# SerezD/gen_adversarial

Hardware: AMD Instinct MI355X
Metric: purified images/sec (attack+encode+decode) (higher is better)
Workload: dtype f32 storage; contractions as 3x bf16 MFMA (hi/lo split), fp32 accumulate; 1 GPU; configs[1]: NVAE purify + VGG-11, 64x64, PGD-Linf step (fwd + input-grad), bs 256 images/GPU x EoT 32 = 8192 defender rows per step, alphas ours_cosine_no_preprocessing_ids.yaml x0.7, assumed NVAE config (C=32, 3x8 groups, 20 latents); images_per_gpu=256, eot=32, rows_per_gpu=8192, chunk_rows=1024, streams=2, parallelism=image-sharded x1

## Files before the change

### gen_adversarial_amd/csrc/dec_cell.hip

```cpp
#include "ga_common.h"
#include "dec_cell_common.h"

namespace ga {

template <int C, int TMW, int NW>
__global__ void __launch_bounds__(64 * NW, NW / 4) dec_cell_fwd_kernel(const ga_dec_cell_desc d, const dc_geom gm) {
    constexpr int NTHR = 64 * NW;
    constexpr int M = 32 * TMW * NW, KS = C / 16, NT = C / 32, SW = M / (NTHR / 8);
    constexpr int BH = TMW == 2 ? 2 : 1, BW = SW / BH;
    using WA = w_chunk<C, true, NTHR>;
    using WB = w_chunk<C, false, NTHR>;
    extern __shared__ __attribute__((aligned(16))) float smem[];
    float* wS = smem;
    float* P1 = smem + 25 * DC_CH;
    const int plane_px = (M >> gm.lhw) * gm.PH * gm.PW;
    __bf16* P2h = reinterpret_cast<__bf16*>(P1 + plane_px * DC_PS);
    __bf16* P2l = P2h + M * DC_LDB;
    __bf16* W1h = P2l + M * DC_LDB;
    __bf16* W1l = W1h + WA::ELEMS;
    __bf16* W2h = W1l + WA::ELEMS;
    __bf16* W2l = W2h + WB::ELEMS;

    const int tid = threadIdx.x, lane = tid & 63, wave = tid >> 6, lrow = lane & 31, lh = lane >> 5;
    const int c4 = tid & 7, strip = tid >> 3;
// ... 211 lines not shown

    WA wa, wq;
    wa.issue(g1h, g1l, C, 0, tid);
    wq.issue(g2h, g2l, C, 0, tid);
    const size_t tap_o = (size_t)(tid < 200 ? (tid >> 3) : 0) * d.Hd + 4 * c4;

    for (int i = tid; i < plane_px * (DC_PS / 4); i += NTHR) reinterpret_cast<floatx4*>(P1)[i] = zero;

    bf16x8 xh[TMW][KS], xl[TMW][KS], gh[TMW][KS], gl[TMW][KS];
#pragma unroll
    for (int i = 0; i < TMW; ++i) {
        const size_t gp = pix0 + wb + i * 32 + lrow;
        const size_t n = gp >> gm.lhw;
        const size_t xp = d.act_rep > 1 ? (((n / (size_t)d.act_rep) << gm.lhw) + (gp & (size_t)(gm.HW - 1))) : gp;
#pragma unroll
        for (int ks = 0; ks < KS; ++ks) {
            const int k = ks * 16 + 8 * lh;
            const float* p = d.x + xp * C + k;
            split8(*reinterpret_cast<const floatx4*>(p), *reinterpret_cast<const floatx4*>(p + 4), xh[i][ks], xl[i][ks]);
            const float* q = d.dout + gp * C + k;
            const float* s = d.pro_scale + n * C + k;
            const float* t = d.pro_shift + n * C + k;
            const floatx4 a = *reinterpret_cast<const floatx4*>(q) * *reinterpret_cast<const floatx4*>(s) + *reinterpret_cast<const floatx4*>(t);
            const floatx4 b = *reinterpret_cast<const floatx4*>(q + 4) * *reinterpret_cast<const floatx4*>(s + 4) + *reinterpret_cast<const floatx4*>(t + 4);
            split8(a, b, gh[i][ks], gl[i][ks]);
        }
    }
    const int p0 = tile_pixel<BH, BW>(strip, gm);
    const int ctr = plane_idx(p0, gm);
    const int win = ctr - 2 * gm.PW - 2;
    int prow[TMW][4];
#pragma unroll
    for (int i = 0; i < TMW; ++i)
#pragma unroll
        for (int q = 0; q < 4; ++q) prow[i][q] = plane_idx(wb + i * 32 + 8 * q + 4 * lh, gm) * DC_PS + lrow;

    const int nch = d.Hd / DC_CH;
    DC_T0
#pragma unroll 1
    for (int ch = 0; ch < nch; ++ch) {
        const int h0 = ch * DC_CH;
        wa.store(W1h, W1l, tid);
        wq.store(W2h, W2l, tid);
        __syncthreads();
        DC_T(0)
        const float b1v = d.b1[h0 + lrow];
        const floatx4 bd4 = *reinterpret_cast<const floatx4*>(d.bd + h0 + 4 * c4);
        const floatx4 taps = *reinterpret_cast<const floatx4*>(d.wd + tap_o + h0);
        const floatx4 tapsT = *reinterpret_cast<const floatx4*>(d.wd_bwd + tap_o + h0);
        __builtin_amdgcn_sched_barrier(0);
        floatx16 t1[TMW];
#pragma unroll
        for (int i = 0; i < TMW; ++i)
#pragma unroll
            for (int r = 0; r < 16; ++r) t1[i][r] = 0.f;
        gemm_resident<TMW, KS>(t1, xh, xl, W1h + lrow * WA::PITCH + 8 * lh, W1l + lrow * WA::PITCH + 8 * lh);
#pragma unroll
        for (int i = 0; i < TMW; ++i)
#pragma unroll
            for (int r = 0; r < 16; ++r) {
                const int row = wb + i * 32 + (r & 3) + 8 * (r >> 2) + 4 * lh;
                const float v = t1[i][r] + b1v;
                const float sg = fast_sigmoid(v);
                P4[row * DC_PS + lrow] = sg * (1.0f + v * (1.0f - sg));
                P1[prow[i][r >> 2] + (r & 3) * DC_PS] = v * sg;
            }
        if (tid < 200) {
            *reinterpret_cast<floatx4*>(wS + (tid >> 3) * DC_CH + 4 * c4) = taps;
            *reinterpret_cast<floatx4*>(wT + (tid >> 3) * DC_CH + 4 * c4) = tapsT;
        }
        DC_T(1)
        __syncthreads();
        DC_T(2)
        floatx4 g2[SW];
        dw_tile<BH, BW>(g2, P1 + win * DC_PS + 4 * c4, wS + 4 * c4, gm.PW);
        DC_T(3)
        floatx16 g[TMW];
#pragma unroll
        for (int i = 0; i < TMW; ++i)
#pragma unroll
            for (int r = 0; r < 16; ++r) g[i][r] = 0.f;
        {
            const __bf16* w2h = W2h + lrow * WA::PITCH + 8 * lh;
            const __bf16* w2l = W2l + lrow * WA::PITCH + 8 * lh;
            constexpr int KPJ = KS / SW;
            bf16x8 bh[KPJ], bl[KPJ];
#pragma unroll
            for (int k = 0; k < KPJ; ++k) {
                bh[k] = *reinterpret_cast<const bf16x8*>(w2h + k * 16);
                bl[k] = *reinterpret_cast<const bf16x8*>(w2l + k * 16);
            }
#pragma unroll
            for (int j = 0; j < SW; ++j) {
                bf16x8 nh[KPJ], nl[KPJ];
                if (j + 1 < SW) {
#pragma unroll
                    for (int k = 0; k < KPJ; ++k) {
                        nh[k] = *reinterpret_cast<const bf16x8*>(w2h + ((j + 1) * KPJ + k) * 16);
                        nl[k] = *reinterpret_cast<const bf16x8*>(w2l + ((j + 1) * KPJ + k) * 16);
                    }
                }
#pragma unroll
                for (int k = 0; k < KPJ; ++k)
#pragma unroll
                    for (int i = 0; i < TMW; ++i) mfma3(g[i], gh[i][j * KPJ + k], gl[i][j * KPJ + k], bh[k], bl[k]);
#pragma unroll
                for (int e = 0; e < 4; ++e) g2[j][e] = dsilu_f(g2[j][e] + bd4[e]);
                interleave_mfma_valu<KPJ * TMW * 3, 44>();
                __builtin_amdgcn_sched_barrier(0);
                if (j + 1 < SW) {
#pragma unroll
                    for (int k = 0; k < KPJ; ++k) { bh[k] = nh[k]; bl[k] = nl[k]; }
                }
            }
        }
        DC_T(4)
        __syncthreads();
        DC_T(5)
        {
            const int h1 = min(h0 + DC_CH, (nch - 1) * DC_CH);
            wa.issue(g1h, g1l, C, h1, tid);
            wq.issue(g2h, g2l, C, h1, tid);
        }
#pragma unroll
        for (int i = 0; i < TMW; ++i)
#pragma unroll
            for (int r = 0; r < 16; ++r) P1[prow[i][r >> 2] + (r & 3) * DC_PS] = g[i][r];
        __syncthreads();
        DC_T(6)
#pragma unroll
        for (int j = 0; j < SW; ++j) {
            floatx4* q = reinterpret_cast<floatx4*>(P1 + (ctr + (j / BW) * gm.PW + (j % BW)) * DC_PS + 4 * c4);
            *q = *q * g2[j];
        }
        __syncthreads();
        DC_T(7)
        {
            floatx4 a[SW];
            dw_tile<BH, BW>(a, P1 + win * DC_PS + 4 * c4, wT + 4 * c4, gm.PW);
#pragma unroll
            for (int j = 0; j < SW; ++j) {
                const int pj = p0 + (j / BW) * gm.W + (j % BW);
                const floatx4 u = *reinterpret_cast<const floatx4*>(P4 + pj * DC_PS + 4 * c4);
                *reinterpret_cast<floatx4*>(d.y + (pix0 + pj) * d.Hd + h0 + 4 * c4) = a[j] * u;
            }
        }
        DC_T(8)
        __syncthreads();
        DC_T(9)
    }
    DC_TEND
}

static int log2_exact(int v) {
    int l = 0;
    while ((1 << l) < v) ++l;
    return (1 << l) == v ? l : -1;
}

constexpr size_t DC_LDS_MAX = 160 * 1024;

static int dc_tile_pixels(int C) { return C == 128 ? 256 : C == 256 ? 128 : 0; }

static size_t dc_lds_bytes(int C, int M, int H, int W, bool bwd) {
    const size_t plane_px = (size_t)(M / (H * W)) * (H + 4) * (W + 4);
    const size_t rows32 = (size_t)2 * 32 * (C + 8) * 2, cols32 = (size_t)2 * C * 40 * 2;
    return bwd ? (size_t)(50 * DC_CH + plane_px * DC_PS + (size_t)M * DC_PS) * 4 + 2 * rows32
               : (size_t)(25 * DC_CH + plane_px * DC_PS) * 4 + (size_t)2 * M * DC_LDB * 2 + rows32 + cols32;
}

template <int C, int TMW, int NW>
static int launch_dec_cell(const ga_dec_cell_desc& d, const dc_geom& gm, hipStream_t stream) {
    constexpr int M = 32 * TMW * NW;
    const size_t lds = dc_lds_bytes(C, M, d.H, d.W, d.backward != 0);
    const dim3 grid((unsigned)((size_t)d.N * d.H * d.W / M));
    if (d.backward) {
        static dyn_lds_cache attr;
        if (!ensure_dyn_lds(attr, reinterpret_cast<const void*>(&dec_cell_bwd_kernel<C, TMW, NW>), lds)) return GA_E_LAUNCH;
        hipLaunchKernelGGL((dec_cell_bwd_kernel<C, TMW, NW>), grid, dim3(64 * NW), lds, stream, d, gm);
    } else {
        static dyn_lds_cache attr;
        if (!ensure_dyn_lds(attr, reinterpret_cast<const void*>(&dec_cell_fwd_kernel<C, TMW, NW>), lds)) return GA_E_LAUNCH;
        hipLaunchKernelGGL((dec_cell_fwd_kernel<C, TMW, NW>), grid, dim3(64 * NW), lds, stream, d, gm);
    }
    return check_launch();
}

}

#ifdef GA_DC_TRACE
extern "C" int ga_debug_dc_trace_read(unsigned long long* out, int n) {
    return hipMemcpyFromSymbol(out, HIP_SYMBOL(ga::ga_dc_trace_buf), (size_t)n * 8) == hipSuccess ? GA_OK : GA_E_LAUNCH;
}
#endif

extern "C" int ga_dec_cell_supported(int N, int H, int W, int C, int Hd) {
    using namespace ga;
    const int M = dc_tile_pixels(C);
    if (!M || N <= 0 || H <= 0 || W <= 0 || Hd <= 0 || Hd % DC_CH) return 0;
    if (log2_exact(W) < 0 || log2_exact(H) < 0) return 0;
    const long HW = (long)H * W;
    if (HW > M || M % HW || W % (M / 32)) return 0;
    if (C == 128 && H % 2) return 0;
    if (((long)N * HW) % M) return 0;
    return dc_lds_bytes(C, M, H, W, true) <= DC_LDS_MAX && dc_lds_bytes(C, M, H, W, false) <= DC_LDS_MAX;
}

extern "C" int ga_dec_cell(const ga_dec_cell_desc* dp, void* stream_) {
    ga::clear_stale_error();
    using namespace ga;
    if (!dp) return GA_E_BADARG;
    const ga_dec_cell_desc& d = *dp;
    if (!d.x || !d.w1_hi || !d.w1_lo || !d.b1 || !d.wd || !d.bd || !d.w2_hi || !d.w2_lo || !d.y) return GA_E_BADARG;
    if (d.backward ? (!d.dout || !d.pro_scale || !d.pro_shift || !d.wd_bwd) : !d.b2) return GA_E_BADARG;
    if (!ga_dec_cell_supported(d.N, d.H, d.W, d.C, d.Hd)) return GA_E_UNSUPPORTED;
    if (d.act_rep > 1 && (!d.backward || d.N % d.act_rep)) return GA_E_BADARG;
    const void* ptrs[] = {d.x, d.w1_hi, d.w1_lo, d.wd, d.wd_bwd, d.bd, d.w2_hi, d.w2_lo, d.dout, d.pro_scale, d.pro_shift, d.y};
    for (const void* p : ptrs) if (p && !aligned16(p)) return GA_E_ALIGN;
    dc_geom gm;
    gm.W = d.W; gm.HW = d.H * d.W; gm.lw = log2_exact(d.W); gm.lhw = log2_exact(gm.HW); gm.PW = d.W + 4; gm.PH = d.H + 4;
    hipStream_t stream = reinterpret_cast<hipStream_t>(stream_);
    if (d.C == 128) return d.variant == 1 ? launch_dec_cell<128, 1, 8>(d, gm, stream) : launch_dec_cell<128, 2, 4>(d, gm, stream);
    if (d.C == 256) return launch_dec_cell<256, 1, 4>(d, gm, stream);
    return GA_E_UNSUPPORTED;
}
```

### gen_adversarial_amd/engine.py

```python
from __future__ import annotations

import ctypes as C
import json
import os
from typing import Dict, List, Optional, Sequence

import torch

from . import _lib as L
from . import folding as F
from .nvae_spec import DecCellSpec, EncCellSpec, NVAESpec, build_spec
from .e4e_spec import E4ESpec
from .resnet_spec import ResNetSpec
from .vgg_spec import VggSpec
from .engine_core import (IMG_LD, RES_SCALE, TILES, TUNE_FILE, WS_FLOATS, Act, WeightStore, _ptr, conv_key,
                          candidate_tiles, resolve_tile, tile_candidates, tune_cache)
from .engine_classifiers import ClassifierBuilder
from .engine_e4e import E4EBuilder
from .engine_avae import AvaeBuilder
from .engine_ndvae import NdvaeBuilder
from .engine_nvae import NvaeBuilder
from .engine_stylegan import StyleGanBuilder
from .engine_trans import TransBuilder


def expand_alpha_rows(alphas, rows: int, rep: int, pairs: bool) -> torch.Tensor:
    t = alphas.detach().to('cpu', torch.float64) if isinstance(alphas, torch.Tensor) else torch.tensor(alphas, dtype=torch.float64)
    if t.dim() != 2:
        raise ValueError(f'a [K, n] table of alpha vectors expected, got shape {tuple(t.shape)}')
    K = t.shape[0]
    if K != rows:
        if K < 1 or rep % K or rows % rep:
            raise ValueError(f'{K} candidates do not divide the {rep} rows per image')
        t = t.repeat_interleave(rep // K, dim=0).repeat(rows // rep, 1)
    if not pairs:
        return t.to(torch.float32)
    return torch.stack([t.to(torch.float32), (1.0 - t).to(torch.float32)], dim=2).reshape(rows, -1)


class Engine(NvaeBuilder, NdvaeBuilder, AvaeBuilder, ClassifierBuilder, E4EBuilder, StyleGanBuilder, TransBuilder):
    fuse_dec_cells = os.environ.get('GA_FUSE_DEC_CELL', '1') != '0'
    fuse_min_workgroups = 0 if os.environ.get('GA_FUSE_DEC_CELL') == 'force' else 160
    fuse_halo_cells = os.environ.get('GA_FUSE_HALO_CELL', '0') == '1'
    dec_cell_variant = int(os.environ.get('GA_DEC_CELL_VARIANT', '1'))

    def __init__(self, nvae_sd, nvae_cfg: dict, resolution, vgg_sd, vgg_spec: VggSpec, rows: int, rep: int,
                 alphas: Sequence[float], temperature: float = 0.6, noise_eps: float = 0.0,
                 device: str = 'cuda:0', need_backward: bool = True, dry_run: bool = False,
                 store: Optional[WeightStore] = None, precision: str = 'bf16x3', blur: bool = False,
                 share_encoder: bool = False, cot_rep: int = 1, alpha_rows: bool = False, alpha_grad: bool = False):
        if rows % rep:
            raise ValueError('rows must be a multiple of the EoT repeat')
        self.device = torch.device(device)
        self.dry_run = dry_run
        if self.device.type != 'cuda' and not dry_run:
            raise RuntimeError('the HIP engine needs a GPU device; there is no CPU fallback '
                               '(dry_run=True only builds and validates the plans)')
        if precision not in ('fp32', 'bf16x3'):
            raise ValueError("precision must be 'fp32' (exact f32 MFMA) or 'bf16x3' (3 bf16 MFMAs per product)")
        self.precision = precision
        self.store = store if store is not None else WeightStore(self.device)
        self.has_nvae = nvae_sd is not None
        self.spec: Optional[NVAESpec] = build_spec(nvae_cfg, resolution) if self.has_nvae else None
        self.resolution = tuple(resolution)
        self.vspec = vgg_spec
        self.rows, self.rep = rows, rep
        self.alphas = [float(a) for a in alphas]
        if self.has_nvae and len(self.alphas) != len(self.spec.groups):
            raise ValueError(f'{len(self.spec.groups)} interpolation alphas expected, got {len(self.alphas)}')
        self.temperature = float(temperature)
        self.noise_eps = float(noise_eps)
        self.blur = bool(blur)
        self._init_alpha_rows(alpha_rows)
        self.share_encoder = bool(share_encoder) and rep > 1 and self.noise_eps == 0.0 and nvae_sd is not None
        self.enc_rows = rows // rep if self.share_encoder else rows
        self.need_backward = need_backward
        if cot_rep < 1:
            raise ValueError('cot_rep (cotangents per forward row of the backward plan) must be at least 1')
        if cot_rep > 1 and not (isinstance(vgg_spec, VggSpec) or (isinstance(vgg_spec, ResNetSpec) and not self.has_nvae)):
            raise ValueError('cot_rep > 1 (K-cotangent backward) is built for the defenders in front of a VGG classifier, for the VGG '
                             'classifier itself and for a bare ResNet / ResNeXt classifier (input noise and blur included); still '
                             'refused: a purifier in front of a ResNet / ResNeXt classifier, and the e4e classifier spec')
        self.cot_rep = int(cot_rep)
        self._init_alpha_grad(alpha_grad)
        self._init_plans()
        self._build(nvae_sd, vgg_sd)

    @classmethod
    def bare(cls, rows: int, device='cuda:0', precision: str = 'bf16x3', store: Optional[WeightStore] = None,
             dry_run: bool = False, rep: int = 1, resolution=None, alphas: Sequence[float] = (), noise_eps: float = 0.0,
             need_backward: bool = True, blur: bool = False, share_encoder: bool = False, alpha_rows: bool = False,
             cot_rep: int = 1, alpha_grad: bool = False) -> "Engine":
        if cot_rep < 1:
            raise ValueError('cot_rep (cotangents per forward row of the backward plan) must be at least 1')
        self = cls.__new__(cls)
        self.device, self.dry_run, self.precision = torch.device(device), dry_run, precision
        if self.device.type != 'cuda' and not dry_run:
            raise RuntimeError('the HIP engine needs a GPU device; there is no CPU fallback')
        self.store = store if store is not None else WeightStore(self.device)
        if rows % rep:
            raise ValueError('rows must be a multiple of the EoT repeat')
        self.has_nvae, self.spec, self.vspec, self.resolution = False, None, None, (tuple(resolution) if resolution else None)
        self.rows, self.rep, self.alphas, self.temperature = rows, rep, [float(a) for a in alphas], 1.0
        self.noise_eps, self.blur = float(noise_eps), bool(blur)
        self._init_alpha_rows(alpha_rows)
        self.share_encoder = bool(share_encoder) and rep > 1 and self.noise_eps == 0.0
        self.enc_rows = rows // rep if self.share_encoder else rows
        self.need_backward, self.image_s2d, self.cot_rep = need_backward, False, int(cot_rep)
        self._init_alpha_grad(alpha_grad)
        self._init_plans()
        self._scratch = {}
        self.eps, self.purified, self.dpurified, self._purified_grad_nhwc = [], None, None, None
        return self

    def finish(self):
        self._finish(0)
        return self

    def _init_plans(self):
        self.bytes = 0
        self.acts = {}
        self.version = 0
        self._sampler_descs = []
        self._keep = []
        self._conv_w = {}
        self.fwd = L.Plan()
        self.bwd = L.Plan()
        self._bwd_steps = []

    def _init_alpha_rows(self, alpha_rows: bool):
        self.alpha_rows, self.alpha_table = bool(alpha_rows), None
        if self.alpha_rows and self.rep > 1 and self.noise_eps != 0.0:
            raise ValueError('a per-row alpha engine with rep > 1 shares the encoder pass of an image between its rows: '
                             'not available with input noise (initial_noise_eps > 0)')

    def _init_alpha_grad(self, alpha_grad: bool):
        self.alpha_grad, self.alpha_grad_rows = bool(alpha_grad), None
        if self.alpha_grad and self.cot_rep > 1:
            raise ValueError('alpha_grad reduces one cotangent per row: not available together with cot_rep > 1')
        if self.alpha_grad and not self.need_backward:
            raise ValueError('alpha_grad lives in the backward plan: not available with need_backward=False')

    def alpha_grads(self) -> torch.Tensor:
        if self.alpha_grad_rows is None:
            raise RuntimeError('engine was built without the alpha-gradient ops (alpha_grad=True)')
        return self.alpha_grad_rows

    def _alloc_alpha_table(self, n: int, pairs: bool) -> torch.Tensor:
        self._alpha_pairs = pairs
        self.alpha_table = self.alloc((self.rows, (2 if pairs else 1) * n))
        self.alpha_table.copy_(expand_alpha_rows([self.alphas], self.rows, self.rows, pairs))
        return self.alpha_table

    def alloc(self, shape) -> torch.Tensor:
        t = torch.zeros(shape, dtype=torch.float32, device=self.device)
        self.bytes += t.numel() * 4
        self._keep.append(t)
        return t

    def dev(self, t: torch.Tensor) -> torch.Tensor:
        t = t.to(self.device, dtype=torch.float32).contiguous()
        self._keep.append(t)
        self.bytes += t.numel() * 4
        return t

    def devd(self, key: str, fn) -> dict:
        return self.store.get(key, fn)

    def conv(self, plan, name, x, w, y, *, cin=None, cout=None, bias=None, K=1, sn=1, sd=1, pad=0,
             x2=None, pro_scale=None, pro_shift=None, pro_act=0, pro_per_row=0,
             addend=None, addend_bcast=False, addend2=None, dact_x=None, dact_scale=None, dact_shift=None, dact_act=0,
             in_hw=None, out_hw=None, n=None, KH=None, KW=None, anchored=False, explicit_out=False,
             ldx=None, ldy=None, ldadd=None, flags=0, precise=False):
        d = L.ConvDesc()
        N, Hi, Wi, Cx = x.shape
        d.x, d.ldx = _ptr(x), (ldx or Cx)
        d.C1 = cin if cin is not None else Cx
        if x2 is not None:
            d.x2, d.ldx2, d.C2 = _ptr(x2), x2.shape[3], x2.shape[3]
        d.w, d.bias = _ptr(w), _ptr(bias)
        if self.precision == 'bf16x3' and not self.dry_run and not precise:
            hi, lo = self.store.split(w)
            d.w_hi, d.w_lo = _ptr(hi), _ptr(lo)
            self._conv_w[id(d)] = w
        d.pro_scale, d.pro_shift, d.pro_act, d.pro_per_row = _ptr(pro_scale), _ptr(pro_shift), pro_act, pro_per_row
        No, Ho, Wo, Cy = y.shape
        d.y, d.ldy = _ptr(y), (ldy or Cy)
        d.flags = flags
        d.Cout = cout if cout is not None else Cy
        if addend is not None:
            d.addend, d.ldadd, d.addend_bcast_n = _ptr(addend), (ldadd or addend.shape[-1]), int(addend_bcast)
        if addend2 is not None:
            d.addend2, d.ldadd2 = _ptr(addend2), addend2.shape[-1]
        if dact_x is not None:
            d.dact_x, d.lddact = _ptr(dact_x), dact_x.shape[-1]
            d.dact_scale, d.dact_shift, d.dact_act = _ptr(dact_scale), _ptr(dact_shift), dact_act
            if dact_x.shape[0] != x.shape[0]:
# ... 403 lines not shown
```

### gen_adversarial_amd/engine_nvae.py

```python
from __future__ import annotations

from typing import Dict, Optional

import torch

from . import _lib as L
from . import folding as F
from .engine_core import IMG_LD, RES_SCALE, Act, _ptr
from .ndvae_spec import NdGenCell, NdResCell
from .nvae_spec import DecCellSpec, EncCellSpec


class NvaeBuilder:
    def enc_cell(self, cell: EncCellSpec, x: Act) -> Act:
        nd = isinstance(cell, NdResCell)
        wts = self.devd(('nd.' if nd else '') + cell.prefix, lambda: (F.fold_nd_res_cell if nd else F.fold_enc_cell)(self.nvae_sd, cell))
        rs = getattr(cell, 'res_scale', RES_SCALE)
        n, h, w = x.n, x.h, x.w
        st = 2 if cell.down else 1
        ho, wo = h // st, w // st
        t1 = Act(self, n, ho, wo, cell.cout, cell.prefix + '.t1')
        t2 = Act(self, n, ho, wo, cell.cout, cell.prefix + '.t2')
        out = Act(self, n, ho, wo, cell.cout, cell.prefix + '.out')
        p = cell.prefix
        self.conv(self.fwd, p + '.conv1', x.t, wts['w1'], t1.t, bias=wts['b1'], K=3, sn=st, pad=1,
                  pro_scale=wts['pro_scale'], pro_shift=wts['pro_shift'], pro_act=L.GA_ACT_SILU)
        self.conv(self.fwd, p + '.conv2', t1.t, wts['w2'], t2.t, bias=wts['b2'], K=3, pad=1, pro_act=L.GA_ACT_SILU)
        if cell.down:
            sk = Act(self, n, ho, wo, cell.cout, p + '.skip')
            ks = 2 if wts['ws'].shape[1] == 4 * x.c else 1
            self.conv(self.fwd, p + '.skip', x.t, wts['ws'], sk.t, bias=wts['bs'], K=ks, sn=2, pad=0, pro_act=L.GA_ACT_SILU)
            skip_t = sk.t
        else:
            skip_t = x.t
        if self.se_merges(t2, ho * wo):
            gate, hid = self.se_forward(p, t2, wts, ho * wo, res_scale=rs, merge=(skip_t, out.t))
        else:
            gate, hid = self.se_forward(p, t2, wts, ho * wo, res_scale=rs)
            a = L.SeApplyDesc()
            a.skip, a.t, a.gate, a.out = _ptr(skip_t), _ptr(t2.t), _ptr(gate), _ptr(out.t)
            a.N, a.H, a.W, a.C, a.skip_mode, a.res_scale = n, ho, wo, cell.cout, 0, rs
            self.fwd.add(a, p + '.merge')

        def backward():
            ps, pb = self.se_backward(p, out.g, t2, wts, gate, hid, ho * wo, res_scale=rs)
            dt1 = self.scratch((out.g.shape[0], ho, wo, cell.cout), 'enc_dt1')
            self.conv(self.bwd, p + '.conv2^T', out.g, wts['w2_bwd'], dt1, K=3, pad=1,
                      pro_scale=ps, pro_shift=pb, pro_per_row=1, dact_x=t1.t, dact_act=L.GA_ACT_SILU)
            if cell.down:
                self.grad_conv_up2(p + '.conv1^T', dt1, wts, 'w1_sub', x, dact_x=x.t, dact_scale=wts['pro_scale'],
                                   dact_shift=wts['pro_shift'], dact_act=L.GA_ACT_SILU)
                self.grad_conv_up2(p + '.skip^T', out.g, wts, 'ws_sub', x, dact_x=x.t, dact_act=L.GA_ACT_SILU)
            else:
                self.grad_conv(p + '.conv1^T', dt1, wts['w1_bwd'], x, K=3, sn=1, sd=1, pad=1, primary=out.g,
                               dact_x=x.t, dact_scale=wts['pro_scale'], dact_shift=wts['pro_shift'], dact_act=L.GA_ACT_SILU)
        self._bwd_steps.append(backward)
        return out

    def dec_cell(self, cell: DecCellSpec, x: Act) -> Act:
        nd = isinstance(cell, NdGenCell)
        wts = self.devd(('nd.' if nd else '') + cell.prefix, lambda: (F.fold_nd_gen_cell if nd else F.fold_dec_cell)(self.nvae_sd, cell))
        rs = getattr(cell, 'res_scale', RES_SCALE)
        n, h, w = x.n, x.h, x.w
        up = cell.up
        H, W = (2 * h, 2 * w) if up else (h, w)
        hid_c = cell.hidden
        p = cell.prefix
        fused = (not up and not nd and self.precision == 'bf16x3' and self.fuse_dec_cells and cell.cout == x.c
                 and L.lib.ga_dec_cell_supported(n, H, W, x.c, hid_c) == 1
                 and n * H * W // (256 if x.c == 128 else 128) >= self.fuse_min_workgroups)
        halo = (not fused and not up and not nd and self.precision == 'bf16x3' and self.fuse_dec_cells
                and (self.fuse_halo_cells or not self.need_backward) and cell.cout == x.c
                and self.cot_rep == 1 and L.lib.ga_dec_cell_halo_supported(n, H, W, x.c, hid_c) == 1
                and n * H * W // 128 >= self.fuse_min_workgroups)
        t3 = Act(self, n, H, W, cell.cout, p + '.t3')
        out = Act(self, n, H, W, cell.cout, p + '.out')

        def halo_desc(backward: int) -> L.DecCellHaloDesc:
            f = L.DecCellHaloDesc()
            f.x, f.b1, f.wd, f.wd_bwd, f.bd, f.b2 = (_ptr(x.t), _ptr(wts['b1']), _ptr(wts['wd']), _ptr(wts['wd_bwd']),
                                                    _ptr(wts['bd']), _ptr(wts['b2']))
            if not self.dry_run:
                (h1, l1), (h2, l2) = self.store.split(wts['w1']), self.store.split(wts['w2_bwd' if backward else 'w2'])
                f.w1_hi, f.w1_lo, f.w2_hi, f.w2_lo = _ptr(h1), _ptr(l1), _ptr(h2), _ptr(l2)
                if backward:
                    h3, l3 = self.store.split(wts['w1_bwd'])
                    f.w1t_hi, f.w1t_lo = _ptr(h3), _ptr(l3)
            f.N, f.H, f.W, f.Cin, f.Cout, f.Hd, f.backward, f.up = n, H, W, x.c, cell.cout, hid_c, backward, 0
            return f

        def fused_desc(backward: int) -> L.DecCellDesc:
            f = L.DecCellDesc()
            f.x, f.b1, f.wd, f.wd_bwd, f.bd, f.b2 = (_ptr(x.t), _ptr(wts['b1']), _ptr(wts['wd']), _ptr(wts['wd_bwd']),
                                                    _ptr(wts['bd']), _ptr(wts['b2']))
            if not self.dry_run:
                (h1, l1), (h2, l2) = self.store.split(wts['w1']), self.store.split(wts['w2_bwd' if backward else 'w2'])
                f.w1_hi, f.w1_lo, f.w2_hi, f.w2_lo = _ptr(h1), _ptr(l1), _ptr(h2), _ptr(l2)
            f.N, f.H, f.W, f.C, f.Hd, f.backward = n, H, W, x.c, hid_c, backward
            f.variant = self.dec_cell_variant if x.c == 128 else 0
            return f

        if fused:
            f = fused_desc(0)
            f.y = _ptr(t3.t)
            self.fwd.add(f, p + '.cell')
        elif halo:
            f = halo_desc(0)
            f.y = _ptr(t3.t)
            self.fwd.add(f, p + '.cell')
        else:
            t1 = Act(self, n, h, w, hid_c, p + '.t1')
            t2 = Act(self, n, H, W, hid_c, p + '.t2')
            self.conv(self.fwd, p + '.pw1', x.t, wts['w1'], t1.t, bias=wts['b1'], K=1)
            d = L.DwDesc()
            d.x, d.w, d.bias, d.y = _ptr(t1.t), _ptr(wts['wd']), _ptr(wts['bd']), _ptr(t2.t)
            d.N, d.H, d.W, d.C, d.pro_act, d.up2 = n, H, W, hid_c, L.GA_ACT_SILU, int(up)
            self.fwd.add(d, p + '.dw5')
            if nd:
                u = t2
                t2 = Act(self, n, H, W, hid_c, p + '.t2p')
                self.conv(self.fwd, p + '.pw', u.t, wts['wp'], t2.t, bias=wts['bp'], K=1)
            self.conv(self.fwd, p + '.pw2', t2.t, wts['w2'], t3.t, bias=wts['b2'], K=1, pro_act=L.GA_ACT_SILU)
        if not up and self.se_merges(t3, H * W):
            gate, hid = self.se_forward(p, t3, wts, H * W, res_scale=rs, merge=(x.t, out.t))
        else:
            a = L.SeApplyDesc()
            if up:
                sl = Act(self, n, h, w, cell.cout, p + '.skip_low')
                self.conv(self.fwd, p + '.skip', x.t, wts['ws'], sl.t, bias=wts['bs'], K=1)
                a.skip, a.skip_mode = _ptr(sl.t), 1
            else:
                a.skip, a.skip_mode = _ptr(x.t), 0
            gate, hid = self.se_forward(p, t3, wts, H * W, res_scale=rs)
            a.t, a.gate, a.out = _ptr(t3.t), _ptr(gate), _ptr(out.t)
            a.N, a.H, a.W, a.C, a.res_scale = n, H, W, cell.cout, rs
            self.fwd.add(a, p + '.merge')

        def backward():
            nc = out.g.shape[0]
            ps, pb = self.se_backward(p, out.g, t3, wts, gate, hid, H * W, res_scale=rs)
            if halo:
                b = halo_desc(1)
                b.dout, b.pro_scale, b.pro_shift, b.addend, b.y = _ptr(out.g), _ptr(ps), _ptr(pb), _ptr(out.g), _ptr(x.g)
                if x.g_written:
                    b.addend2 = _ptr(x.g)
                self.bwd.add(b, p + '.cell^T')
                x.g_written = True
                return
            dt1 = self.scratch((nc, h, w, hid_c), 'dec_dt1')
            if fused:
                b = fused_desc(1)
                b.dout, b.pro_scale, b.pro_shift, b.y = _ptr(out.g), _ptr(ps), _ptr(pb), _ptr(dt1)
                b.N, b.act_rep = nc, self.cot_rep
                self.bwd.add(b, p + '.cell^T')
            else:
                dt2 = self.scratch((nc, H, W, hid_c), 'dec_dt2')
                self.conv(self.bwd, p + '.pw2^T', out.g, wts['w2_bwd'], dt2, K=1,
                          pro_scale=ps, pro_shift=pb, pro_per_row=1, dact_x=t2.t, dact_act=L.GA_ACT_SILU)
                if nd:
                    du = self.scratch((nc, H, W, hid_c), 'dec_du')
                    self.conv(self.bwd, p + '.pw^T', dt2, wts['wp_bwd'], du, K=1)
                    dt2 = du
                b = L.DwDesc()
                b.x, b.w, b.dact_x, b.y = _ptr(dt2), _ptr(wts['wd_bwd']), _ptr(t1.t), _ptr(dt1)
                b.N, b.H, b.W, b.C, b.dact_act, b.pool2, b.act_rep = nc, H, W, hid_c, L.GA_ACT_SILU, int(up), self.cot_rep
                self.bwd.add(b, p + '.dw5^T')
            self.grad_conv(p + '.pw1^T', dt1, wts['w1_bwd'], x, K=1, primary=None if up else out.g)
            if up:
                dsl = self.scratch((nc, h, w, cell.cout), 'dec_dsl')
                bl = L.BilinearBwdDesc()
                bl.dhigh, bl.dlow, bl.N, bl.h, bl.w, bl.C, bl.accumulate = _ptr(out.g), _ptr(dsl), nc, h, w, cell.cout, 0
                self.bwd.add(bl, p + '.bilinear^T')
                self.grad_conv(p + '.skip^T', dsl, wts['ws_bwd'], x, K=1)
        self._bwd_steps.append(backward)
        return out

    def _build_nvae(self, x0: Act) -> Act:
        nvae_sd = self.nvae_sd
        spec, R = self.spec, self.rows
        H = spec.resolution
        NL = spec.num_latent
        self.latent_pitch = (NL + 7) // 8 * 8
        self.eps = [self.alloc((R, NL, gs.res, gs.res)) for gs in spec.groups]
        self.purified = self.alloc((R, 3, H, H))
        if self.alpha_rows:
            self._alloc_alpha_table(len(spec.groups), pairs=True)
        if self.alpha_grad:
            self.alpha_grad_rows = self.alloc((R, len(spec.groups)))

        stem = self.devd('stem', lambda: F.pad_image_conv(F.fold_wn_conv(nvae_sd, 'preprocessing_block.init_conv'), 3, IMG_LD))
        norm = self.devd('norm05', lambda: {'two': torch.full((IMG_LD,), 2.0), 'mone': torch.full((IMG_LD,), -1.0)})
        two, mone = norm['two'], norm['mone']
        RE = self.enc_rows
        erep = self.rep if self.share_encoder else 1
        x = Act(self, RE, H, H, spec.base_channels, 'stem')
        self.conv(self.fwd, 'stem', x0.t, stem['w'], x.t, bias=stem['b'], K=3, pad=1, pro_scale=two, pro_shift=mone)
        stem_out = x

        def bwd_stem():
            self.grad_conv('stem^T', stem_out.g, stem['w_bwd'], x0, K=3, pad=1,
                           dact_x=x0.t, dact_scale=two, dact_shift=mone, dact_act=L.GA_ACT_NONE)
        self._bwd_steps.append(bwd_stem)

        for cell in spec.pre_cells:
            x = self.enc_cell(cell, x)

        stash: Dict[str, Act] = {}
        for kind, payload in spec.enc_program:
            if kind == 'stash':
                stash[payload] = x
            else:
                x = self.enc_cell(payload, x)
        x_top = x

        C0 = spec.enc0_channels
        g0 = spec.groups[0]
        enc0 = self.devd('encoder_0', lambda: F.fold_wn_conv(nvae_sd, 'encoder_0.1'))
        e0 = Act(self, RE, g0.res, g0.res, C0, 'enc0')
        self.conv(self.fwd, 'encoder_0', x_top.t, enc0['w'], e0.t, bias=enc0['b'], K=1, pro_act=L.GA_ACT_ELU)
        NLP = self.latent_pitch
        s00 = self.devd('enc_sampler_0:0', lambda: F.pad_conv_out(
            F.fold_wn_conv(nvae_sd, 'enc_sampler.sampler_0:0', out_slice=slice(0, NL)), NL, NLP))
        muq0 = Act(self, RE, g0.res, g0.res, NLP, 'mu_q0')
        self.conv(self.fwd, 'enc_sampler_0:0', e0.t, s00['w'], muq0.t, bias=s00['b'], K=3, pad=1, pro_act=L.GA_ACT_ELU)
        z = Act(self, R, g0.res, g0.res, NLP, 'z0')
        self._sampler_fwd('sample_0:0', muq0, None, self.eps[0], z, self.alphas[0], q_rep=erep)

        def fold_comb0():
            wfull = F.wn_weight64(nvae_sd, 'decoder_combiners.combiner_0:0.conv')[:, :, 0, 0]
            prior = nvae_sd['const_prior'].double()[0]
            pc = torch.einsum('oc,chw->hwo', wfull[:, :C0], prior) + \
                nvae_sd['decoder_combiners.combiner_0:0.conv.bias'].double()
            if spec.num_nf_cells:
                pc = pc - wfull[:, C0:] @ F.nf_constant_shift(nvae_sd, '0:0', spec.num_nf_cells, NL)
            return {'pc': pc.float().unsqueeze(0), 'wz': F.pad_cols(wfull[:, C0:].float(), 0, NL, NLP),
                    'wz_bwd': F.pad_rows(wfull[:, C0:].t().float().contiguous(), NLP)}
        c0w = self.devd('combiner_0:0', fold_comb0)
        pc, wz, wz_bwd = c0w['pc'], c0w['wz'], c0w['wz_bwd']
        x = Act(self, R, g0.res, g0.res, C0, 'comb_0:0')
        self.conv(self.fwd, 'combiner_0:0', z.t, wz, x.t, K=1, addend=pc, addend_bcast=True)
        comb0_out, z0 = x, z

        def bwd_group0():
            self.grad_conv('combiner_0:0^T', comb0_out.g, wz_bwd, z0, K=1)
            self._sampler_bwd('sample_0:0^T', muq0, None, self.eps[0], z0, self.alphas[0], None, q_rep=erep)
            self.grad_conv('enc_sampler_0:0^T', muq0.g, s00['w_bwd'], e0, K=3, pad=1, dact_x=e0.t, dact_act=L.GA_ACT_ELU)
            self.grad_conv('encoder_0^T', e0.g, enc0['w_bwd'], x_top, K=1, dact_x=x_top.t, dact_act=L.GA_ACT_ELU)
        group0_bwd = bwd_group0

        dec_bwd_steps_start = len(self._bwd_steps)
        self._bwd_steps.append(group0_bwd)

# ... 155 lines not shown
```

Baseline: 6323 defender rows/s (rows = images x EoT-32).

## Add warp-specialized pair kernels for C=256 fused decoder cells

Adds forward and backward fused decoder-cell kernels for C=256 that run 512 threads per block, split into two wave groups. One group runs the first pointwise GEMM and the other runs the second GEMM or depthwise work, with the stages overlapping across hidden-channel chunks. The goal is more concurrent MFMA and VALU work per workgroup and better latency hiding than the single-group 256-thread kernel. These kernels become the default for both passes through a new environment tuple. The cost is added code complexity and a possible occupancy or LDS-pressure change.

```diff
diff --git a/gen_adversarial_amd/csrc/dec_cell.hip b/gen_adversarial_amd/csrc/dec_cell.hip
--- a/gen_adversarial_amd/csrc/dec_cell.hip
+++ b/gen_adversarial_amd/csrc/dec_cell.hip
@@ -387,6 +387,459 @@
     DC_TEND
 }
 
+__device__ __forceinline__ void dc_silu_split_store(const floatx4 t2, __bf16* ph, __bf16* pl) {
+    floatx4 v = t2;
+#pragma unroll
+    for (int e = 0; e < 4; ++e) v[e] = silu_f(v[e]);
+    bf16x4 hi, lo;
+    split4(v, hi, lo);
+    *reinterpret_cast<bf16x4*>(ph) = hi;
+    *reinterpret_cast<bf16x4*>(pl) = lo;
+}
+
+template <int C>
+__global__ void __launch_bounds__(512, 2) dec_cell_fwd_pair_kernel(const ga_dec_cell_desc d, const dc_geom gm) {
+    constexpr int NTHR = 512, M = 128, KS = C / 16, NT = C / 32, SW = 2;
+    using WA = w_chunk<C, true, NTHR>;
+    using WB = w_chunk<C, false, NTHR>;
+    extern __shared__ __attribute__((aligned(16))) float smem[];
+    float* wS = smem;
+    float* P1 = smem + 25 * DC_CH;
+    const int plane_px = (M >> gm.lhw) * gm.PH * gm.PW;
+    __bf16* P2h = reinterpret_cast<__bf16*>(P1 + plane_px * DC_PS);
+    __bf16* P2l = P2h + M * DC_LDB;
+    __bf16* W1h = P2l + M * DC_LDB;
+    __bf16* W1l = W1h + WA::ELEMS;
+    __bf16* W2h = W1l + WA::ELEMS;
+    __bf16* W2l = W2h + WB::ELEMS;
+
+    const int tid = threadIdx.x, lane = tid & 63, lrow = lane & 31, lh = lane >> 5;
+    const int wave = __builtin_amdgcn_readfirstlane(tid >> 6);
+    const int c4 = tid & 7, strip = (tid & 255) >> 3, half = tid >> 8;
+    const size_t pix0 = (size_t)blockIdx.x * M;
+    const int wb = (wave & 3) * 32;
+    const floatx4 zero = {0.f, 0.f, 0.f, 0.f};
+    const __bf16* g1h = reinterpret_cast<const __bf16*>(d.w1_hi);
+    const __bf16* g1l = reinterpret_cast<const __bf16*>(d.w1_lo);
+    const __bf16* g2h = reinterpret_cast<const __bf16*>(d.w2_hi);
+    const __bf16* g2l = reinterpret_cast<const __bf16*>(d.w2_lo);
+    const int nch = d.Hd / DC_CH;
+    const int last = (nch - 1) * DC_CH;
+
+    WA wa;
+    WB wq;
+    for (int i = tid; i < plane_px * (DC_PS / 4); i += NTHR) reinterpret_cast<floatx4*>(P1)[i] = zero;
+
+    const int p0 = strip_pixel<2 * SW>(strip, gm) + SW * half;
+    const float* dwin = P1 + (plane_idx(p0, gm) - 2 * gm.PW - 2) * DC_PS + 4 * c4;
+    __bf16* p2h = P2h + p0 * DC_LDB + 4 * c4;
+    __bf16* p2l = P2l + p0 * DC_LDB + 4 * c4;
+
+    if (wave < 4) {
+        __builtin_amdgcn_sched_barrier(0);
+        wa.issue(g1h, g1l, C, 0, tid);
+        wq.issue(g2h, g2l, d.Hd, 0, tid);
+        const int tap_o = (tid < 200 ? (tid >> 3) : 0) * d.Hd + 4 * c4;
+        floatx4 taps = *reinterpret_cast<const floatx4*>(d.wd + tap_o);
+        bf16x8 xh[1][KS], xl[1][KS];
+#pragma unroll
+        for (int ks = 0; ks < KS; ++ks) {
+            const float* p = d.x + (pix0 + wb + lrow) * C + ks * 16 + 8 * lh;
+            split8(*reinterpret_cast<const floatx4*>(p), *reinterpret_cast<const floatx4*>(p + 4), xh[0][ks], xl[0][ks]);
+        }
+        int prow[4];
+#pragma unroll
+        for (int q = 0; q < 4; ++q) prow[q] = plane_idx(wb + 8 * q + 4 * lh, gm) * DC_PS + lrow;
+        const __bf16* w1h = W1h + lrow * WA::PITCH + 8 * lh;
+        const __bf16* w1l = W1l + lrow * WA::PITCH + 8 * lh;
+
+        wa.store(W1h, W1l, tid);
+        wq.store(W2h, W2l, tid);
+        if (tid < 200) *reinterpret_cast<floatx4*>(wS + (tid >> 3) * DC_CH + 4 * c4) = taps;
+        __syncthreads();
+        wa.issue(g1h, g1l, C, min(DC_CH, last), tid);
+        floatx16 t1[1];
+#pragma unroll
+        for (int r = 0; r < 16; ++r) t1[0][r] = 0.f;
+        gemm_resident<1, KS>(t1, xh, xl, w1h, w1l);
+        {
+            const float b1v = d.b1[lrow];
+#pragma unroll
+            for (int r = 0; r < 16; ++r) P1[prow[r >> 2] + (r & 3) * DC_PS] = silu_f(t1[0][r] + b1v);
+        }
+        __syncthreads();
+        wa.store(W1h, W1l, tid);
+        __syncthreads();
+
+        DC_T0
+#pragma unroll 1
+        for (int ch = 0; ch < nch; ++ch) {
+            const int h0 = ch * DC_CH;
+            const int h1 = min(h0 + DC_CH, last), h2 = min(h0 + 2 * DC_CH, last);
+            const float b1v = d.b1[h1 + lrow];
+            const floatx4 bd4 = *reinterpret_cast<const floatx4*>(d.bd + h0 + 4 * c4);
+            __builtin_amdgcn_sched_barrier(0);
+            wa.issue(g1h, g1l, C, h2, tid);
+            wq.issue(g2h, g2l, d.Hd, h1, tid);
+            floatx4 a[SW];
+            dw_strip<SW>(a, dwin, wS + 4 * c4, gm.PW);
+            DC_T(0)
+#pragma unroll
+            for (int r = 0; r < 16; ++r) t1[0][r] = 0.f;
+            {
+                constexpr int NR = 8, KPR = KS / NR;
+                bf16x8 bh[KPR], bl[KPR];
+#pragma unroll
+                for (int k = 0; k < KPR; ++k) {
+                    bh[k] = *reinterpret_cast<const bf16x8*>(w1h + k * 16);
+                    bl[k] = *reinterpret_cast<const bf16x8*>(w1l + k * 16);
+                }
+#pragma unroll
+                for (int rg = 0; rg < NR; ++rg) {
+                    bf16x8 nh[KPR], nl[KPR];
+                    if (rg + 1 < NR) {
+#pragma unroll
+                        for (int k = 0; k < KPR; ++k) {
+                            nh[k] = *reinterpret_cast<const bf16x8*>(w1h + ((rg + 1) * KPR + k) * 16);
+                            nl[k] = *reinterpret_cast<const bf16x8*>(w1l + ((rg + 1) * KPR + k) * 16);
+                        }
+                    }
+#pragma unroll
+                    for (int k = 0; k < KPR; ++k) mfma3(t1[0], xh[0][rg * KPR + k], xl[0][rg * KPR + k], bh[k], bl[k]);
+                    if (rg % (NR / SW) == 0) {
+                        const int j = rg / (NR / SW);
+                        dc_silu_split_store(a[j] + bd4, p2h + j * DC_LDB, p2l + j * DC_LDB);
+                        interleave_mfma_valu<KPR * 3, 42>();
+                    }
+                    __builtin_amdgcn_sched_barrier(0);
+                    if (rg + 1 < NR) {
+#pragma unroll
+                        for (int k = 0; k < KPR; ++k) { bh[k] = nh[k]; bl[k] = nl[k]; }
+                    }
+                }
+            }
+            DC_T(1)
+            __syncthreads();
+            wa.store(W1h, W1l, tid);
+            taps = *reinterpret_cast<const floatx4*>(d.wd + tap_o + h1);
+            DC_T(2)
+#pragma unroll
+            for (int r = 0; r < 16; ++r) P1[prow[r >> 2] + (r & 3) * DC_PS] = silu_f(t1[0][r] + b1v);
+            DC_T(3)
+            if (tid < 200) *reinterpret_cast<floatx4*>(wS + (tid >> 3) * DC_CH + 4 * c4) = taps;
+            __syncthreads();
+            wq.store(W2h, W2l, tid);
+            DC_T(4)
+        }
+        DC_TEND
+    } else {
+        wa.issue(g1h, g1l, C, 0, tid);
+        wq.issue(g2h, g2l, d.Hd, 0, tid);
+        floatx16 acc[NT];
+#pragma unroll
+        for (int j = 0; j < NT; ++j)
+#pragma unroll
+            for (int r = 0; r < 16; ++r) acc[j][r] = 0.f;
+        const __bf16* w2h = W2h + lrow * WB::PITCH + 8 * lh;
+        const __bf16* w2l = W2l + lrow * WB::PITCH + 8 * lh;
+        const int a_o = (wb + lrow) * DC_LDB + 8 * lh;
+
+        wa.store(W1h, W1l, tid);
+        wq.store(W2h, W2l, tid);
+        __syncthreads();
+        wa.issue(g1h, g1l, C, min(DC_CH, last), tid);
+        __syncthreads();
+        wa.store(W1h, W1l, tid);
+        __syncthreads();
+
+        DC_T0
+#pragma unroll 1
+        for (int ch = 0; ch < nch; ++ch) {
+            const int h0 = ch * DC_CH;
+            const int h1 = min(h0 + DC_CH, last), h2 = min(h0 + 2 * DC_CH, last);
+            const floatx4 bd4 = *reinterpret_cast<const floatx4*>(d.bd + h0 + 4 * c4);
+            __builtin_amdgcn_sched_barrier(0);
+            wa.issue(g1h, g1l, C, h2, tid);
+            wq.issue(g2h, g2l, d.Hd, h1, tid);
+            floatx4 a[SW];
+            dw_strip<SW>(a, dwin, wS + 4 * c4, gm.PW);
+            DC_T(0)
+#pragma unroll
+            for (int j = 0; j < SW; ++j) dc_silu_split_store(a[j] + bd4, p2h + j * DC_LDB, p2l + j * DC_LDB);
+            DC_T(1)
+            __syncthreads();
+            wa.store(W1h, W1l, tid);
+            DC_T(2)
+            {
+                bf16x8 ah[2], al[2];
+#pragma unroll
+                for (int ks = 0; ks < 2; ++ks) {
+                    ah[ks] = *reinterpret_cast<const bf16x8*>(P2h + a_o + ks * 16);
+                    al[ks] = *reinterpret_cast<const bf16x8*>(P2l + a_o + ks * 16);
+                }
+                constexpr int NG = 2 * NT;
+                bf16x8 bh = *reinterpret_cast<const bf16x8*>(w2h), bl = *reinterpret_cast<const bf16x8*>(w2l);
+#pragma unroll
+                for (int g = 0; g < NG; ++g) {
+                    bf16x8 nh, nl;
+                    if (g + 1 < NG) {
+                        nh = *reinterpret_cast<const bf16x8*>(w2h + ((g + 1) >> 1) * 32 * WB::PITCH + ((g + 1) & 1) * 16);
+                        nl = *reinterpret_cast<const bf16x8*>(w2l + ((g + 1) >> 1) * 32 * WB::PITCH + ((g + 1) & 1) * 16);
+                    }
+                    mfma3(acc[g >> 1], ah[g & 1], al[g & 1], bh, bl);
+                    __builtin_amdgcn_sched_barrier(0);
+                    if (g + 1 < NG) { bh = nh; bl = nl; }
+                }
+            }
+            DC_T(3)
+            __syncthreads();
+            wq.store(W2h, W2l, tid);
+            DC_T(4)
+        }
+        DC_TEND
+#pragma unroll
+        for (int j = 0; j < NT; ++j) {
+            const float b2v = d.b2[j * 32 + lrow];
+#pragma unroll
+            for (int r = 0; r < 16; ++r) {
+                const int row = wb + (r & 3) + 8 * (r >> 2) + 4 * lh;
+                d.y[(pix0 + row) * C + j * 32 + lrow] = acc[j][r] + b2v;
+            }
+        }
+    }
+}
+
+template <int C>
+__global__ void __launch_bounds__(512, 2) dec_cell_bwd_pair_kernel(const ga_dec_cell_desc d, const dc_geom gm) {
+    constexpr int NTHR = 512, M = 128, KS = C / 16, SW = 2;
+    using WA = w_chunk<C, true, NTHR>;
+    extern __shared__ __attribute__((aligned(16))) float smem[];
+    float* wS = smem;
+    float* wT = smem + 25 * DC_CH;
+    float* P1 = smem + 50 * DC_CH;
+    const int plane_px = (M >> gm.lhw) * gm.PH * gm.PW;
+    float* P4 = P1 + plane_px * DC_PS;
+    __bf16* W1h = reinterpret_cast<__bf16*>(P4 + M * DC_PS);
+    __bf16* W1l = W1h + WA::ELEMS;
+    __bf16* W2h = W1l + WA::ELEMS;
+    __bf16* W2l = W2h + WA::ELEMS;
+
+    const int tid = threadIdx.x, lane = tid & 63, lrow = lane & 31, lh = lane >> 5;
+    const int wave = __builtin_amdgcn_readfirstlane(tid >> 6);
+    const int c4 = tid & 7, strip = (tid & 255) >> 3, half = tid >> 8;
+    const size_t pix0 = (size_t)blockIdx.x * M;
+    const int wb = (wave & 3) * 32;
+    const floatx4 zero = {0.f, 0.f, 0.f, 0.f};
+    const __bf16* g1h = reinterpret_cast<const __bf16*>(d.w1_hi);
+    const __bf16* g1l = reinterpret_cast<const __bf16*>(d.w1_lo);
+    const __bf16* g2h = reinterpret_cast<const __bf16*>(d.w2_hi);
+    const __bf16* g2l = reinterpret_cast<const __bf16*>(d.w2_lo);
+
+    WA wa, wq;
+    for (int i = tid; i < plane_px * (DC_PS / 4); i += NTHR) reinterpret_cast<floatx4*>(P1)[i] = zero;
+
+    const int p0 = strip_pixel<2 * SW>(strip, gm) + SW * half;
+    const int ctr = plane_idx(p0, gm);
+    const float* dwin = P1 + (ctr - 2 * gm.PW - 2) * DC_PS + 4 * c4;
+    float* own = P1 + ctr * DC_PS + 4 * c4;
+    const float* p4 = P4 + p0 * DC_PS + 4 * c4;
+    int prow[4];
+#pragma unroll
+    for (int q = 0; q < 4; ++q) prow[q] = plane_idx(wb + 8 * q + 4 * lh, gm) * DC_PS + lrow;
+    const int nch = d.Hd / DC_CH;
+    const int lastc = (nch - 1) * DC_CH;
+
+    auto dsilu2 = [&](floatx4 (&g2)[SW], const floatx4 bd4) {
+#pragma unroll
+        for (int j = 0; j < SW; ++j)
+#pragma unroll
+            for (int e = 0; e < 4; ++e) g2[j][e] = dsilu_f(g2[j][e] + bd4[e]);
+    };
+    auto scale_own = [&](const floatx4 (&g2)[SW]) {
+#pragma unroll
+        for (int j = 0; j < SW; ++j) {
+            floatx4* q = reinterpret_cast<floatx4*>(own + j * DC_PS);
+            *q = *q * g2[j];
+        }
+    };
+    auto dwT_store = [&](const int h0) {
+        floatx4 a[SW];
+        dw_strip<SW>(a, dwin, wT + 4 * c4, gm.PW);
+#pragma unroll
+        for (int j = 0; j < SW; ++j) {
+            const floatx4 u = *reinterpret_cast<const floatx4*>(p4 + j * DC_PS);
+            *reinterpret_cast<floatx4*>(d.y + (pix0 + p0 + j) * d.Hd + h0 + 4 * c4) = a[j] * u;
+        }
+    };
+
+    if (wave < 4) {
+        __builtin_amdgcn_sched_barrier(0);
+        wa.issue(g1h, g1l, C, 0, tid);
+        wq.issue(g2h, g2l, C, 0, tid);
+        bf16x8 xh[1][KS], xl[1][KS];
+        {
+            const size_t gp = pix0 + wb + lrow;
+            const size_t n = gp >> gm.lhw;
+            const size_t xp = d.act_rep > 1 ? (((n / (size_t)d.act_rep) << gm.lhw) + (gp & (size_t)(gm.HW - 1))) : gp;
+#pragma unroll
+            for (int ks = 0; ks < KS; ++ks) {
+                const float* p = d.x + xp * C + ks * 16 + 8 * lh;
+                split8(*reinterpret_cast<const floatx4*>(p), *reinterpret_cast<const floatx4*>(p + 4), xh[0][ks], xl[0][ks]);
+            }
+        }
+        DC_T0
+#pragma unroll 1
+        for (int ch = 0; ch < nch; ++ch) {
+            const int h0 = ch * DC_CH;
+            wa.store(W1h, W1l, tid);
+            wq.store(W2h, W2l, tid);
+            __syncthreads();
+            DC_T(0)
+            const float b1v = d.b1[h0 + lrow];
+            const floatx4 bd4 = *reinterpret_cast<const floatx4*>(d.bd + h0 + 4 * c4);
+            __builtin_amdgcn_sched_barrier(0);
+            floatx16 t1[1];
+#pragma unroll
+            for (int r = 0; r < 16; ++r) t1[0][r] = 0.f;
+            gemm_resident<1, KS>(t1, xh, xl, W1h + lrow * WA::PITCH + 8 * lh, W1l + lrow * WA::PITCH + 8 * lh);
+#pragma unroll
+            for (int r = 0; r < 16; ++r) {
+                const int row = wb + (r & 3) + 8 * (r >> 2) + 4 * lh;
+                const float v = t1[0][r] + b1v;
+                const float sg = fast_sigmoid(v);
+                P4[row * DC_PS + lrow] = sg * (1.0f + v * (1.0f - sg));
+                P1[prow[r >> 2] + (r & 3) * DC_PS] = v * sg;
+            }
+            DC_T(1)
+            __syncthreads();
+            DC_T(2)
+            floatx4 g2[SW];
+            dw_strip<SW>(g2, dwin, wS + 4 * c4, gm.PW);
+            DC_T(3)
+            dsilu2(g2, bd4);
+            DC_T(4)
+            __syncthreads();
+            DC_T(5)
+            {
+                const int h1 = min(h0 + DC_CH, lastc);
+                wa.issue(g1h, g1l, C, h1, tid);
+                wq.issue(g2h, g2l, C, h1, tid);
+            }
+            __syncthreads();
+            DC_T(6)
+            scale_own(g2);
+            __syncthreads();
+            DC_T(7)
+            dwT_store(h0);
+            DC_T(8)
+            __syncthreads();
+            DC_T(9)
+        }
+        DC_TEND
+    } else {
+        wa.issue(g1h, g1l, C, 0, tid);
+        wq.issue(g2h, g2l, C, 0, tid);
+        bf16x8 gh[1][KS], gl[1][KS];
+        {
+            const size_t gp = pix0 + wb + lrow;
+            const size_t n = gp >> gm.lhw;
+#pragma unroll
+            for (int ks = 0; ks < KS; ++ks) {
+                const int k = ks * 16 + 8 * lh;
+                const float* q = d.dout + gp * C + k;
+                const float* s = d.pro_scale + n * C + k;
+                const float* t = d.pro_shift + n * C + k;
+                const floatx4 a = *reinterpret_cast<const floatx4*>(q) * *reinterpret_cast<const floatx4*>(s) + *reinterpret_cast<const floatx4*>(t);
+                const floatx4 b = *reinterpret_cast<const floatx4*>(q + 4) * *reinterpret_cast<const floatx4*>(s + 4) + *reinterpret_cast<const floatx4*>(t + 4);
+                split8(a, b, gh[0][ks], gl[0][ks]);
+            }
+        }
+        const int ttid = tid - 256;
+        const size_t tap_o = (size_t)(ttid < 200 ? (ttid >> 3) : 0) * d.Hd + 4 * c4;
+        const __bf16* w2h = W2h + lrow * WA::PITCH + 8 * lh;
+        const __bf16* w2l = W2l + lrow * WA::PITCH + 8 * lh;
+        DC_T0
+#pragma unroll 1
+        for (int ch = 0; ch < nch; ++ch) {
+            const int h0 = ch * DC_CH;
+            wa.store(W1h, W1l, tid);
+            wq.store(W2h, W2l, tid);
+            __syncthreads();
+            DC_T(0)
+            const floatx4 bd4 = *reinterpret_cast<const floatx4*>(d.bd + h0 + 4 * c4);
+            const floatx4 taps = *reinterpret_cast<const floatx4*>(d.wd + tap_o + h0);
+            const floatx4 tapsT = *reinterpret_cast<const floatx4*>(d.wd_bwd + tap_o + h0);
+            __builtin_amdgcn_sched_barrier(0);
+            if (ttid < 200) {
+                *reinterpret_cast<floatx4*>(wS + (ttid >> 3) * DC_CH + 4 * c4) = taps;
+                *reinterpret_cast<floatx4*>(wT + (ttid >> 3) * DC_CH + 4 * c4) = tapsT;
+            }
+            DC_T(1)
+            __syncthreads();
+            DC_T(2)
+            floatx4 g2[SW];
+            dw_strip<SW>(g2, dwin, wS + 4 * c4, gm.PW);
+            DC_T(3)
+            floatx16 g[1];
+#pragma unroll
+            for (int r = 0; r < 16; ++r) g[0][r] = 0.f;
+            {
+                constexpr int NR = 8, KPR = KS / NR;
+                bf16x8 bh[KPR], bl[KPR];
+#pragma unroll
+                for (int k = 0; k < KPR; ++k) {
+                    bh[k] = *reinterpret_cast<const bf16x8*>(w2h + k * 16);
+                    bl[k] = *reinterpret_cast<const bf16x8*>(w2l + k * 16);
+                }
+#pragma unroll
+                for (int rg = 0; rg < NR; ++rg) {
+                    bf16x8 nh[KPR], nl[KPR];
+                    if (rg + 1 < NR) {
+#pragma unroll
+                        for (int k = 0; k < KPR; ++k) {
+                            nh[k] = *reinterpret_cast<const bf16x8*>(w2h + ((rg + 1) * KPR + k) * 16);
+                            nl[k] = *reinterpret_cast<const bf16x8*>(w2l + ((rg + 1) * KPR + k) * 16);
+                        }
+                    }
+#pragma unroll
+                    for (int k = 0; k < KPR; ++k) mfma3(g[0], gh[0][rg * KPR + k], gl[0][rg * KPR + k], bh[k], bl[k]);
+                    if (rg % (NR / SW) == 0) {
+                        const int j = rg / (NR / SW);
+#pragma unroll
+                        for (int e = 0; e < 4; ++e) g2[j][e] = dsilu_f(g2[j][e] + bd4[e]);
+                        interleave_mfma_valu<KPR * 3, 44>();
+                    }
+                    __builtin_amdgcn_sched_barrier(0);
+                    if (rg + 1 < NR) {
+#pragma unroll
+                        for (int k = 0; k < KPR; ++k) { bh[k] = nh[k]; bl[k] = nl[k]; }
+                    }
+                }
+            }
+            DC_T(4)
+            __syncthreads();
+            DC_T(5)
+            {
+                const int h1 = min(h0 + DC_CH, lastc);
+                wa.issue(g1h, g1l, C, h1, tid);
+                wq.issue(g2h, g2l, C, h1, tid);
+            }
+#pragma unroll
+            for (int r = 0; r < 16; ++r) P1[prow[r >> 2] + (r & 3) * DC_PS] = g[0][r];
+            __syncthreads();
+            DC_T(6)
+            scale_own(g2);
+            __syncthreads();
+            DC_T(7)
+            dwT_store(h0);
+            DC_T(8)
+            __syncthreads();
+            DC_T(9)
+        }
+        DC_TEND
+    }
+}
+
 static int log2_exact(int v) {
     int l = 0;
     while ((1 << l) < v) ++l;
@@ -421,6 +874,23 @@
     return check_launch();
 }
 
+template <int C>
+static int launch_dec_cell_pair(const ga_dec_cell_desc& d, const dc_geom& gm, hipStream_t stream) {
+    constexpr int M = 128;
+    const size_t lds = dc_lds_bytes(C, M, d.H, d.W, d.backward != 0);
+    const dim3 grid((unsigned)((size_t)d.N * d.H * d.W / M));
+    if (d.backward) {
+        static dyn_lds_cache attr;
+        if (!ensure_dyn_lds(attr, reinterpret_cast<const void*>(&dec_cell_bwd_pair_kernel<C>), lds)) return GA_E_LAUNCH;
+        hipLaunchKernelGGL((dec_cell_bwd_pair_kernel<C>), grid, dim3(512), lds, stream, d, gm);
+    } else {
+        static dyn_lds_cache attr;
+        if (!ensure_dyn_lds(attr, reinterpret_cast<const void*>(&dec_cell_fwd_pair_kernel<C>), lds)) return GA_E_LAUNCH;
+        hipLaunchKernelGGL((dec_cell_fwd_pair_kernel<C>), grid, dim3(512), lds, stream, d, gm);
+    }
+    return check_launch();
+}
+
 }
 
 #ifdef GA_DC_TRACE
@@ -450,12 +920,13 @@
     if (d.backward ? (!d.dout || !d.pro_scale || !d.pro_shift || !d.wd_bwd) : !d.b2) return GA_E_BADARG;
     if (!ga_dec_cell_supported(d.N, d.H, d.W, d.C, d.Hd)) return GA_E_UNSUPPORTED;
     if (d.act_rep > 1 && (!d.backward || d.N % d.act_rep)) return GA_E_BADARG;
+    if (d.variant != 0 && d.variant != 1) return GA_E_UNSUPPORTED;
     const void* ptrs[] = {d.x, d.w1_hi, d.w1_lo, d.wd, d.wd_bwd, d.bd, d.w2_hi, d.w2_lo, d.dout, d.pro_scale, d.pro_shift, d.y};
     for (const void* p : ptrs) if (p && !aligned16(p)) return GA_E_ALIGN;
     dc_geom gm;
     gm.W = d.W; gm.HW = d.H * d.W; gm.lw = log2_exact(d.W); gm.lhw = log2_exact(gm.HW); gm.PW = d.W + 4; gm.PH = d.H + 4;
     hipStream_t stream = reinterpret_cast<hipStream_t>(stream_);
     if (d.C == 128) return d.variant == 1 ? launch_dec_cell<128, 1, 8>(d, gm, stream) : launch_dec_cell<128, 2, 4>(d, gm, stream);
-    if (d.C == 256) return launch_dec_cell<256, 1, 4>(d, gm, stream);
+    if (d.C == 256) return d.variant == 1 ? launch_dec_cell_pair<256>(d, gm, stream) : launch_dec_cell<256, 1, 4>(d, gm, stream);
     return GA_E_UNSUPPORTED;
 }
diff --git a/gen_adversarial_amd/engine.py b/gen_adversarial_amd/engine.py
--- a/gen_adversarial_amd/engine.py
+++ b/gen_adversarial_amd/engine.py
@@ -43,6 +43,7 @@
     fuse_min_workgroups = 0 if os.environ.get('GA_FUSE_DEC_CELL') == 'force' else 160
     fuse_halo_cells = os.environ.get('GA_FUSE_HALO_CELL', '0') == '1'
     dec_cell_variant = int(os.environ.get('GA_DEC_CELL_VARIANT', '1'))
+    dec_cell_variant_c256 = tuple(int(v) for v in os.environ.get('GA_DEC_CELL_VARIANT_C256', '11'))
 
     def __init__(self, nvae_sd, nvae_cfg: dict, resolution, vgg_sd, vgg_spec: VggSpec, rows: int, rep: int,
                  alphas: Sequence[float], temperature: float = 0.6, noise_eps: float = 0.0,
diff --git a/gen_adversarial_amd/engine_nvae.py b/gen_adversarial_amd/engine_nvae.py
--- a/gen_adversarial_amd/engine_nvae.py
+++ b/gen_adversarial_amd/engine_nvae.py
@@ -97,7 +97,7 @@
                 (h1, l1), (h2, l2) = self.store.split(wts['w1']), self.store.split(wts['w2_bwd' if backward else 'w2'])
                 f.w1_hi, f.w1_lo, f.w2_hi, f.w2_lo = _ptr(h1), _ptr(l1), _ptr(h2), _ptr(l2)
             f.N, f.H, f.W, f.C, f.Hd, f.backward = n, H, W, x.c, hid_c, backward
-            f.variant = self.dec_cell_variant if x.c == 128 else 0
+            f.variant = self.dec_cell_variant if x.c == 128 else self.dec_cell_variant_c256[backward] if x.c == 256 else 0
             return f
 
         if fused:
```

Result: no change. 6356 defender rows/s (rows = images x EoT-32), median of 6 (+0.5%).
